# paolomandica/HALO

Measured on AMD Instinct MI355X. Metric: acquisition-scored images/sec (1024x2048, C=256, 19 cls), higher is better.
Workload: dtype f64

## Files before the change

### halo_amd/csrc/halo_score.hip

```cpp
#include "halo_common.hpp"
#include "halo_devmath.hpp"
#include "halo_select_plan.hpp"
#include "halo_softmax.hpp"
#include <stdlib.h>
#include <type_traits>

namespace halo {

constexpr int TPB = 256;
#ifndef HALO_FTPB
#define HALO_FTPB 128
#endif
#ifndef HALO_FEAT_WAVES
#define HALO_FEAT_WAVES 4
#endif
#ifndef HALO_FEAT_UNROLL
#define HALO_FEAT_UNROLL 8
#endif
#ifndef HALO_FEAT_STORE
#define HALO_FEAT_STORE 2
#endif
#ifndef HALO_FEAT_ENT_STORE
#define HALO_FEAT_ENT_STORE 1
#endif
// ... 765 lines not shown
    const int X0 = blockIdx.x * WB_TW, Y0 = blockIdx.y * WB_TH;
    const int nrows = H - Y0 < WB_TH ? H - Y0 : WB_TH, ncols = W - X0 < WB_TW ? W - X0 : WB_TW;
    const int Wt = WB_TW + 2 * r, Ht = nrows + 2 * r;
    const long long hw = (long long)H * W;
    const float *ep = ent + (size_t)b * hw;
    {
        const int tx = tid & 127;
        if (tx < Wt) {
            const int xs = tile_src(X0 + tx - r, W, X0 + ncols - 1, r, pad);
            for (int ty = tid >> 7; ty < Ht; ty += TPB / 128) {
                const int ys = tile_src(Y0 + ty - r, H, Y0 + nrows - 1, r, pad);
                tile[ty][tx] = (xs >= 0 && ys >= 0) ? ep[(size_t)ys * W + xs] : 0.0f;
            }
        }
    }
    __syncthreads();
    const int ry = tid & (WB_TH - 1), lx = (tid / WB_TH) * WB_P;
    const int y = Y0 + ry, xb = X0 + lx;
    const bool live = ry < nrows && lx < ncols;
    double mn = 0.0, mx = 0.0;
    if (live) {
        const int nfull = k >> 2, rem = k & 3;
        float acc[WB_P];
#pragma unroll
        for (int j = 0; j < WB_P; ++j) acc[j] = 0.0f;
        for (int dy = 0; dy < k; ++dy) {
            const float4 *row = reinterpret_cast<const float4 *>(&tile[ry + dy][lx]);
            float v[12];
            { const float4 q = row[0]; v[0] = q.x; v[1] = q.y; v[2] = q.z; v[3] = q.w; }
            { const float4 q = row[1]; v[4] = q.x; v[5] = q.y; v[6] = q.z; v[7] = q.w; }
            for (int c = 0; c < nfull; ++c) {
                { const float4 q = row[c + 2]; v[8] = q.x; v[9] = q.y; v[10] = q.z; v[11] = q.w; }
#pragma unroll
                for (int t = 0; t < 4; ++t)
#pragma unroll
                    for (int j = 0; j < WB_P; ++j) acc[j] = acc[j] + v[j + t];
#pragma unroll
                for (int i = 0; i < 8; ++i) v[i] = v[i + 4];
            }
#pragma unroll
            for (int j = 0; j < WB_P; ++j) acc[j] = acc[j] + v[j];
            if (rem == 3) {
                const float4 q = row[nfull + 2];
                v[8] = q.x; v[9] = q.y;
#pragma unroll
                for (int t = 1; t < 3; ++t)
#pragma unroll
                    for (int j = 0; j < WB_P; ++j) acc[j] = acc[j] + v[j + t];
            }
        }
        bool have = false;
#pragma unroll
        for (int j = 0; j < WB_P; ++j) {
            const int x = xb + j;
            if (x < W) {
                float cnt = 1.0f;
                if (pk > 0 && pad) {
                    cnt = (float)(pk * pk);
                } else if (pk > 0) {
                    const int pr = pk / 2;
                    const int y0 = y - pr < 0 ? 0 : y - pr, y1 = y + pr >= H ? H - 1 : y + pr;
                    const int x0 = x - pr < 0 ? 0 : x - pr, x1 = x + pr >= W ? W - 1 : x + pr;
                    cnt = (float)((y1 - y0 + 1) * (x1 - x0 + 1));
                }
                const float a = acc[j] / cnt;
                unc[(size_t)b * hw + (size_t)y * W + x] = a;
                if (!have) { mn = mx = (double)a; have = true; }
                else { mn = nan_min(mn, (double)a); mx = nan_max(mx, (double)a); }
            }
        }
    }
    if (!partials) return;
    __shared__ double seed[2];
    if (tid == 0) { seed[0] = mn; seed[1] = mx; }
    __syncthreads();
    if (!live) { mn = seed[0]; mx = seed[1]; }
    block_minmax<TPB>(mn, mx, partials + (((size_t)b * gridDim.y + blockIdx.y) * gridDim.x + blockIdx.x) * 2);
}

__device__ __forceinline__ float lane_prev(float v)
{
    return __int_as_float(__builtin_amdgcn_update_dpp(0, __float_as_int(v), 0x138 , 0xf, 0xf, false));
}
__device__ __forceinline__ float lane_next(float v)
{
    return __int_as_float(__builtin_amdgcn_update_dpp(0, __float_as_int(v), 0x130 , 0xf, 0xf, false));
}

__device__ __forceinline__ float box3_over_count(float a, int H, int W, int y, int xx, int pk)
{
    if (pk <= 0) return a;
    const int rr = pk / 2;
    const int y0 = y - rr < 0 ? 0 : y - rr, y1 = y + rr >= H ? H - 1 : y + rr;
    const int x0 = xx - rr < 0 ? 0 : xx - rr, x1 = xx + rr >= W ? W - 1 : xx + rr;
    return a / (float)((y1 - y0 + 1) * (x1 - x0 + 1));
}

__device__ __forceinline__ void box3_row4(const float *__restrict__ ep, int H, int W, int y, int x, bool live, int pk, float (&o)[4])
{
    const int lane = threadIdx.x & 63;
    float r[3][6];
#pragma unroll
    for (int dy = 0; dy < 3; ++dy) {
        const int yy = y + dy - 1;
        const bool in = live && yy >= 0 && yy < H;
        const float *row = ep + (size_t)(in ? yy : 0) * W;
        float4 q = make_float4(0.0f, 0.0f, 0.0f, 0.0f);
        if (in) q = *reinterpret_cast<const float4 *>(row + x);
        float left = lane_prev(q.w), right = lane_next(q.x);
        if (lane == 0) left = (in && x > 0) ? row[x - 1] : 0.0f;
        if (lane == 63) right = (in && x + 4 < W) ? row[x + 4] : 0.0f;
        r[dy][0] = (in && x > 0) ? left : 0.0f;
        r[dy][1] = q.x; r[dy][2] = q.y; r[dy][3] = q.z; r[dy][4] = q.w;
        r[dy][5] = (in && x + 4 < W) ? right : 0.0f;
    }
#pragma unroll
    for (int j = 0; j < 4; ++j) {
        float a = 0.0f;
#pragma unroll
        for (int dy = 0; dy < 3; ++dy)
#pragma unroll
            for (int dx = 0; dx < 3; ++dx) a = a + r[dy][j + dx];
        o[j] = box3_over_count(a, H, W, y, x + j, pk);
    }
}

__global__ void __launch_bounds__(TPB) k_box3_unc(const float *__restrict__ ent, int H, int W, int pk,
                                                  float *__restrict__ unc, double *__restrict__ partials)
{
    const int b = blockIdx.y;
    const long long hw = (long long)H * W;
    const long long i0 = ((long long)blockIdx.x * TPB + threadIdx.x) * 4;
    const bool live = i0 < hw;
    double mn = 0.0, mx = 0.0;
    const int y = live ? (int)(i0 / W) : 0, x = live ? (int)(i0 % W) : 0;
    float o[4];
    box3_row4(ent + (size_t)b * hw, H, W, y, x, live, pk, o);
    if (live) {
        if (unc) *reinterpret_cast<float4 *>(unc + (size_t)b * hw + i0) = make_float4(o[0], o[1], o[2], o[3]);
        mn = mx = (double)o[0];
#pragma unroll
        for (int j = 1; j < 4; ++j) { mn = nan_min(mn, (double)o[j]); mx = nan_max(mx, (double)o[j]); }
    }
    if (!partials) return;
    __shared__ double seed[2];
    if (threadIdx.x == 0) { seed[0] = mn; seed[1] = mx; }
    __syncthreads();
    if (!live) { mn = seed[0]; mx = seed[1]; }
    block_minmax<TPB>(mn, mx, partials + ((size_t)b * gridDim.x + blockIdx.x) * 2);
}

constexpr int BM_RPT = 4, BM_TW = 256, BM_TH = BM_RPT * (TPB / 64);

__device__ __forceinline__ float nan_minf(float a, float b) { return (a != a) ? a : ((b != b) ? b : (b < a ? b : a)); }
__device__ __forceinline__ float nan_maxf(float a, float b) { return (a != a) ? a : ((b != b) ? b : (b > a ? b : a)); }

__global__ void __launch_bounds__(TPB) k_box3_minmax(const float *__restrict__ ent, int H, int W, int pk, double *__restrict__ partials,
                                                     unsigned *__restrict__ hist_zero)
{
    const int b = blockIdx.z, lane = threadIdx.x & 63, wv = threadIdx.x >> 6;
    if (hist_zero) {
        const unsigned nb = gridDim.x * gridDim.y;
        for (unsigned l = blockIdx.y * gridDim.x + blockIdx.x; l < NB1 / TPB; l += nb) hist_zero[(size_t)b * NB1 + l * TPB + threadIdx.x] = 0u;
    }
    const int x = blockIdx.x * BM_TW + lane * 4, y0 = blockIdx.y * BM_TH + wv * BM_RPT;
    const float *ep = ent + (size_t)b * H * W;
    const bool xin = x < W;
    auto load_row = [&](int yy, float (&r)[6]) {
        const bool in = xin && yy >= 0 && yy < H;
        const float *row = ep + (size_t)(in ? yy : 0) * W;
        float4 q = make_float4(0.0f, 0.0f, 0.0f, 0.0f);
        if (in) q = *reinterpret_cast<const float4 *>(row + x);
        float left = lane_prev(q.w), right = lane_next(q.x);
        if (lane == 0) left = (in && x > 0) ? row[x - 1] : 0.0f;
        if (lane == 63) right = (in && x + 4 < W) ? row[x + 4] : 0.0f;
        r[0] = (in && x > 0) ? left : 0.0f;
        r[1] = q.x; r[2] = q.y; r[3] = q.z; r[4] = q.w;
        r[5] = (in && x + 4 < W) ? right : 0.0f;
    };
    float r0[6], r1[6], r2[6];
    load_row(y0 - 1, r0);
    load_row(y0, r1);
    float mn = 0.0f, mx = 0.0f;
    bool have = false;
#pragma unroll
    for (int k = 0; k < BM_RPT; ++k) {
        const int y = y0 + k;
        load_row(y + 1, r2);
        if (xin && y < H) {
#pragma unroll
            for (int j = 0; j < 4; ++j) {
                float a = 0.0f;
#pragma unroll
                for (int dx = 0; dx < 3; ++dx) a = a + r0[j + dx];
#pragma unroll
                for (int dx = 0; dx < 3; ++dx) a = a + r1[j + dx];
#pragma unroll
                for (int dx = 0; dx < 3; ++dx) a = a + r2[j + dx];
                const float o = box3_over_count(a, H, W, y, x + j, pk);
                if (!have) { mn = mx = o; have = true; }
                else { mn = nan_minf(mn, o); mx = nan_maxf(mx, o); }
            }
        }
#pragma unroll
        for (int q = 0; q < 6; ++q) { r0[q] = r1[q]; r1[q] = r2[q]; }
    }
    __shared__ float seedf[2];
    __shared__ float smn[TPB / 64], smx[TPB / 64];
    if (threadIdx.x == 0) { seedf[0] = mn; seedf[1] = mx; }
    __syncthreads();
    if (!have) { mn = seedf[0]; mx = seedf[1]; }
#pragma unroll
    for (int off = 32; off > 0; off >>= 1) {
        mn = nan_minf(mn, __shfl_xor(mn, off));
        mx = nan_maxf(mx, __shfl_xor(mx, off));
    }
    if (lane == 0) { smn[wv] = mn; smx[wv] = mx; }
    __syncthreads();
    if (threadIdx.x == 0) {
#pragma unroll
        for (int i = 1; i < TPB / 64; ++i) { mn = nan_minf(mn, smn[i]); mx = nan_maxf(mx, smx[i]); }
        double *out2 = partials + (((size_t)b * gridDim.y + blockIdx.y) * gridDim.x + blockIdx.x) * 2;
        out2[0] = (double)mn;
        out2[1] = (double)mx;
    }
}

__global__ void __launch_bounds__(TPB) k_minmax_f32(const float *__restrict__ x, long long hw,
                                                    double *__restrict__ partials)
{
    const int b = blockIdx.y;
    const long long i = (long long)blockIdx.x * TPB + threadIdx.x;
    const bool live = i < hw;
    double mn = 0.0, mx = 0.0;
    if (live) mn = mx = (double)x[(size_t)b * hw + i];
    __shared__ double seed[2];
    if (threadIdx.x == 0) { seed[0] = mn; seed[1] = mx; }
    __syncthreads();
    if (!live) { mn = seed[0]; mx = seed[1]; }
    block_minmax<TPB>(mn, mx, partials + ((size_t)b * gridDim.x + blockIdx.x) * 2);
}

__global__ void __launch_bounds__(TPB) k_fill_f32(float *__restrict__ x, long long n, float v)
{
    const long long i = (long long)blockIdx.x * TPB + threadIdx.x;
    if (i < n) x[i] = v;
}

template <typename TI>
__global__ void __launch_bounds__(TPB) k_combine(const TI *__restrict__ imp_raw, const float *__restrict__ unc_raw,
                                                 const double *__restrict__ stats, const unsigned char *__restrict__ active,
                                                 long long hw, int normalize, TI *__restrict__ score,
                                                 TI *__restrict__ imp_out, float *__restrict__ unc_out)
{
    const int b = blockIdx.y;
    const long long i = (long long)blockIdx.x * TPB + threadIdx.x;
    if (i >= hw) return;
    const size_t o = (size_t)b * hw + i;
    TI im = imp_raw[o];
    float un = unc_raw[o];
    if (normalize) {
        const float umn = (float)stats[b * 4 + 2], umx = (float)stats[b * 4 + 3];
        un = (un - umn) / (float)((double)umx - (double)umn);
        const TI imn = (TI)stats[b * 4 + 0], imx = (TI)stats[b * 4 + 1];
        if constexpr (sizeof(TI) == 8) im = (im - imn) / (imx - imn);
        else im = (im - imn) / (float)((double)imx - (double)imn);
    }
    TI s = im * (TI)un;
    if (active && active[o]) {
        if constexpr (sizeof(TI) == 8) s = __longlong_as_double(0xfff0000000000000ll);
        else s = __uint_as_float(0xff800000u);
    }
    score[o] = s;
    if (imp_out) imp_out[o] = im;
    if (unc_out) unc_out[o] = un;
}


constexpr int CB_ROWS = 16;

template <typename TI>
__global__ void __launch_bounds__(TPB) k_combine_box3(const TI *__restrict__ imp_raw, const float *__restrict__ ent,
                                                      const double *__restrict__ stats, const unsigned char *__restrict__ active,
                                                      int H, int W, int pk, int normalize, TI *__restrict__ score,
                                                      TI *__restrict__ imp_out, float *__restrict__ unc_out, SelHdr *__restrict__ rng,
                                                      unsigned *__restrict__ hist, int rows)
{
    __shared__ unsigned hl[NB1];
    const int b = blockIdx.z;
    const long long hw = (long long)H * W;
    const int x = (blockIdx.x * TPB + threadIdx.x) * 4;
    const bool live = x < W;
    float umn = 0.0f, uden = 1.0f;
    TI imn = (TI)0, iden = (TI)1;
    bool fin = false;
    if (normalize) {
        umn = (float)stats[b * 4 + 2];
        const float umx = (float)stats[b * 4 + 3];
        uden = (float)((double)umx - (double)umn);
        imn = (TI)stats[b * 4 + 0];
        const TI imx = (TI)stats[b * 4 + 1];
        if constexpr (sizeof(TI) == 8) iden = imx - imn;
        else iden = (float)((double)imx - (double)imn);
        fin = uden > 0.0f && uden < __builtin_inff() && iden > (TI)0 && iden < (TI)__builtin_inf();
        if (rng && blockIdx.x == 0 && blockIdx.y == 0 && threadIdx.x == 0) {
            SelHdr h;
            memset(&h, 0, sizeof(h));
            h.kmin_inv = ~order_key(0.0);
            h.kmax = order_key(1.0);
            h.nvalid = 1u;
            h.flags = fin ? (hist ? (unsigned)SEL_F_HIST : 0u) : (unsigned)SEL_F_BAD;
            rng[b] = h;
        }
    }
    const bool count = hist != nullptr && fin;
    if (count) {
        for (int j = threadIdx.x; j < NB1; j += TPB) hl[j] = 0u;
        __syncthreads();
    }
    ValRange vr;
    vr.lo = 0.0; vr.scale = (double)NB1; vr.ok = true;
    const int ybeg = blockIdx.y * rows, yend = ybeg + rows < H ? ybeg + rows : H;
    const float *ep = ent + (size_t)b * hw;
    const int lane = threadIdx.x & 63;
    struct RowRaw { float4 q; float el, er; bool in; };
    auto row_issue = [&](int yy) {
        RowRaw t;
        t.in = live && yy >= 0 && yy < H;
        const float *row = ep + (size_t)(t.in ? yy : 0) * W;
        t.q = make_float4(0.0f, 0.0f, 0.0f, 0.0f);
        t.el = 0.0f; t.er = 0.0f;
        if (t.in) t.q = *reinterpret_cast<const float4 *>(row + x);
        if (lane == 0 && t.in && x > 0) t.el = row[x - 1];
        if (lane == 63 && t.in && x + 4 < W) t.er = row[x + 4];
        return t;
    };
    auto row_finish = [&](const RowRaw &t, float (&r)[6]) {
        float left = lane_prev(t.q.w), right = lane_next(t.q.x);
        if (lane == 0) left = t.el;
        if (lane == 63) right = t.er;
        r[0] = (t.in && x > 0) ? left : 0.0f;
        r[1] = t.q.x; r[2] = t.q.y; r[3] = t.q.z; r[4] = t.q.w;
        r[5] = (t.in && x + 4 < W) ? right : 0.0f;
    };
    typedef double cb_d2 __attribute__((ext_vector_type(2)));
    typedef float cb_f4 __attribute__((ext_vector_type(4)));
    struct PixRaw { cb_d2 d0, d1; cb_f4 f; unsigned am; };
    auto pix_issue = [&](int yy) {
        PixRaw t;
        t.d0 = (cb_d2){0.0, 0.0}; t.d1 = t.d0; t.f = (cb_f4){0.f, 0.f, 0.f, 0.f}; t.am = 0u;
        if (!live || yy >= yend) return t;
        const size_t o = (size_t)b * hw + (size_t)yy * W + x;
        if constexpr (sizeof(TI) == 8) {
            t.d0 = *reinterpret_cast<const cb_d2 *>(imp_raw + o);
            t.d1 = *reinterpret_cast<const cb_d2 *>(imp_raw + o + 2);
        } else {
            t.f = *reinterpret_cast<const cb_f4 *>(imp_raw + o);
        }
        if (active) t.am = *reinterpret_cast<const unsigned *>(active + o);
        return t;
    };
    float r0[6], r1[6], r2[6];
    {
        const RowRaw a0 = row_issue(ybeg - 1), a1 = row_issue(ybeg);
        row_finish(a0, r0);
        row_finish(a1, r1);
    }
    RowRaw nrow = row_issue(ybeg + 1);
    PixRaw npix = pix_issue(ybeg);
    for (int y = ybeg; y < yend; ++y) {
        row_finish(nrow, r2);
        const PixRaw cpix = npix;
        nrow = row_issue(y + 2);
        npix = pix_issue(y + 1);
        float un[4];
#pragma unroll
        for (int j = 0; j < 4; ++j) {
            float a = 0.0f;
#pragma unroll
            for (int dx = 0; dx < 3; ++dx) a = a + r0[j + dx];
#pragma unroll
            for (int dx = 0; dx < 3; ++dx) a = a + r1[j + dx];
#pragma unroll
            for (int dx = 0; dx < 3; ++dx) a = a + r2[j + dx];
            un[j] = box3_over_count(a, H, W, y, x + j, pk);
        }
#pragma unroll
        for (int q = 0; q < 6; ++q) { r0[q] = r1[q]; r1[q] = r2[q]; }
        if (!live) continue;
        const size_t o = (size_t)b * hw + (size_t)y * W + x;
        TI im[4];
        if constexpr (sizeof(TI) == 8) { im[0] = cpix.d0.x; im[1] = cpix.d0.y; im[2] = cpix.d1.x; im[3] = cpix.d1.y; }
        else { im[0] = cpix.f.x; im[1] = cpix.f.y; im[2] = cpix.f.z; im[3] = cpix.f.w; }
        if (normalize) {
#pragma unroll
            for (int j = 0; j < 4; ++j) { un[j] = (un[j] - umn) / uden; im[j] = (im[j] - imn) / iden; }
        }
        const unsigned am = cpix.am;
        TI sc[4];
#pragma unroll
        for (int j = 0; j < 4; ++j) {
            sc[j] = im[j] * (TI)un[j];
            if ((am >> (8 * j)) & 0xffu) {
                if constexpr (sizeof(TI) == 8) sc[j] = __longlong_as_double(0xfff0000000000000ll);
                else sc[j] = __uint_as_float(0xff800000u);
            }
        }
        if (count) {
#pragma unroll
            for (int j = 0; j < 4; ++j) {
                const double v = (double)sc[j];
                const unsigned long long k = order_key(v);
                if (k < KEY_POS_INF && k != KEY_NEG_INF) {
                    double t;
                    atomicAdd(&hl[coarse_bin(v, vr, t)], 1u);
                }
            }
        }
        if constexpr (sizeof(TI) == 8) {
            *reinterpret_cast<double2 *>(score + o) = make_double2(sc[0], sc[1]);
            *reinterpret_cast<double2 *>(score + o + 2) = make_double2(sc[2], sc[3]);
            if (imp_out) {
                *reinterpret_cast<double2 *>(imp_out + o) = make_double2(im[0], im[1]);
                *reinterpret_cast<double2 *>(imp_out + o + 2) = make_double2(im[2], im[3]);
            }
        } else {
            *reinterpret_cast<float4 *>(score + o) = make_float4(sc[0], sc[1], sc[2], sc[3]);
            if (imp_out) *reinterpret_cast<float4 *>(imp_out + o) = make_float4(im[0], im[1], im[2], im[3]);
        }
        if (unc_out) *reinterpret_cast<float4 *>(unc_out + o) = make_float4(un[0], un[1], un[2], un[3]);
    }
    if (count) {
        __syncthreads();
        unsigned *g = hist + (size_t)b * NB1;
        for (int j = threadIdx.x; j < NB1; j += TPB)
            if (hl[j]) atomicAdd(&g[j], hl[j]);
    }
}



constexpr int LR_STAGE_IT = 3, LR_STAGE_G = 4;
constexpr int LR_TW = 64, LR_TH = 16, LR_PPT = 4;

template <typename T, int NPX = LR_PPT> struct LrW { T lx0, lx1, ly0[NPX], ly1[NPX]; };

struct LrTile { unsigned id; int b, X0, Y0; };
template <int TH> __device__ __forceinline__ LrTile lr_tile()
{
    const unsigned ntx = gridDim.x, nty = gridDim.y, ntiles = ntx * nty * gridDim.z;
    const unsigned lin = blockIdx.x + ntx * (blockIdx.y + nty * blockIdx.z);
    const unsigned xq = ntiles / 8, xr = ntiles % 8, xk = lin % 8;
    const unsigned id = (xk < xr ? xk * (xq + 1) : xr * (xq + 1) + (xk - xr) * xq) + lin / 8;
    return {id, (int)(id / (ntx * nty)), (int)(id % ntx) * LR_TW, (int)((id / ntx) % nty) * TH};
// ... 998 lines not shown
    p.pad = (a.flags >> 8) & 3;
    p.normalize = a.flags & HALO_FLAG_NORMALIZE;
    p.hw = (long long)a.H * a.W;
    p.nblk1 = (int)cdiv(p.hw, TPB);
    p.nblk_imp = p.nblk_unc = p.nblk1;

    Arena ar(a.workspace, a.workspace_bytes);
    p.ent = ar.take<float>(B * p.hw);
    p.unc_raw = ar.take<float>(B * p.hw);
    p.imp_raw = ar.take<double>(B * p.hw);
    p.pred = ar.take<short>(B * p.hw);
    p.part_imp = ar.take<double>(B * partial_slots(a.H, a.W) * 2);
    p.part_unc = ar.take<double>(B * partial_slots(a.H, a.W) * 2);
    p.stats = ar.take<double>(B * 4);
    p.lr_logit_full = (p.lr && !(a.O == 19 || a.O == 16)) ? ar.take<float>(B * a.O * p.hw) : nullptr;
    const bool gram_mode = a.route == HALO_SCORE_LR_GRAM && p.need_feat;
    if (gram_mode && a.feat_dtype != HALO_F64) return fail(HALO_E_UNSUPPORTED, "halo_score: float64 embeddings only on the Gram route");
    p.gram = gram_mode ? ar.take<double>(B * GRAM_MAPS * a.hf * a.wf) : nullptr;
    if (!ar.ok()) return fail(HALO_E_WORKSPACE, "halo_score: workspace too small");

    p.f64out = (a.pur_type == HALO_PUR_RADIUS || a.pur_type == HALO_PUR_EUC_NORM) && a.feat_dtype == HALO_F64;
    p.hist = is_ripu(a.pur_type) || a.pur_type == HALO_PUR_HYPER;
    p.mode = a.pur_type == HALO_PUR_EUC_NORM ? 1 : 0;
    p.ks = sqrt(fabs(-a.c) + 1e-15);
    p.rks = 1.0 / p.ks;

    const bool ent_only = (a.unc_type == HALO_UNC_ENTROPY || a.unc_type == HALO_UNC_PIXEL_ENTROPY) && !is_ripu(a.pur_type);
    const int fvec = !p.need_feat ? 0 : (a.feat_dtype == HALO_F64
        ? (((p.hw % 2 == 0) && (a.feat_bstride % 2 == 0) && aligned16(a.feat) && aligned16(p.imp_raw)) ? 2 : 1)
        : (((p.hw % 4 == 0) && (a.feat_bstride % 4 == 0) && aligned16(a.feat) && aligned16(p.imp_raw)) ? 4 : 1));
    p.fuse = !p.lr && p.need_feat && ent_only && (a.O == 19 || a.O == 16) && fvec > 1 && (a.logit_bstride % fvec == 0) &&
             (((uintptr_t)a.logit) % (4 * fvec) == 0);
    p.fl = FusedLogit{a.logit, (long long)a.logit_bstride, (int)a.O, a.unc_type, p.ent};
    return HALO_OK;
}

static void launch_logit_pass(const halo_score_args &a, const ScorePlan &p, hipStream_t st)
{
    if (p.fuse) return;
    const int B = (int)a.B, O = (int)a.O, H = (int)a.H, W = (int)a.W;
    const long long hw = p.hw, bstride = a.logit_bstride;
    const long long *gt = (const long long *)a.gt;
    short *pred = is_ripu(a.pur_type) ? p.pred : nullptr;
    const dim3 block(TPB), grid1((unsigned)p.nblk1, (unsigned)B);
    if (a.unc_type == HALO_UNC_ZEROS && !is_ripu(a.pur_type)) {
        hipLaunchKernelGGL(k_fill_f32, dim3((unsigned)cdiv(B * hw, TPB)), block, 0, st, p.ent, (long long)(B * hw), 0.0f);
    } else if (p.lr) {
        const int hl = (int)a.hl, wl = (int)a.wl;
        const float shl = H > 1 ? (float)(hl - 1) / (float)(H - 1) : 0.0f, swl = W > 1 ? (float)(wl - 1) / (float)(W - 1) : 0.0f;
        if (O == 19)
            hipLaunchKernelGGL((k_logit_maps_lr<19>), grid1, block, 0, st, a.logit, bstride, hl, wl, H, W, shl, swl, gt, a.unc_type, a.pur_type, p.ent, pred);
        else if (O == 16)
            hipLaunchKernelGGL((k_logit_maps_lr<16>), grid1, block, 0, st, a.logit, bstride, hl, wl, H, W, shl, swl, gt, a.unc_type, a.pur_type, p.ent, pred);
        else {
            hipLaunchKernelGGL(k_logit_interp_lr, grid1, block, 0, st, a.logit, bstride, O, hl, wl, H, W, shl, swl, p.lr_logit_full);
            hipLaunchKernelGGL(k_logit_maps_generic, grid1, block, 0, st, (const float *)p.lr_logit_full, (long long)(O * hw), gt, O, hw, a.unc_type, a.pur_type, 0, p.ent, pred);
        }
    } else {
        const bool vec4 = (hw % 4 == 0) && (bstride % 4 == 0) && aligned16(a.logit) && aligned16(p.ent);
        const dim3 grid4((unsigned)cdiv(hw, TPB * 4), (unsigned)B);
        if (O == 19 && vec4)
            hipLaunchKernelGGL((k_logit_maps<19, 4>), grid4, block, 0, st, a.logit, bstride, gt, hw, a.unc_type, a.pur_type, p.ent, pred);
        else if (O == 16 && vec4)
            hipLaunchKernelGGL((k_logit_maps<16, 4>), grid4, block, 0, st, a.logit, bstride, gt, hw, a.unc_type, a.pur_type, p.ent, pred);
        else
            hipLaunchKernelGGL(k_logit_maps_generic, grid1, block, 0, st, a.logit, bstride, gt, O, hw, a.unc_type, a.pur_type, 0, p.ent, pred);
    }
}

static void launch_gram(const halo_score_args &a, const ScorePlan &p, hipStream_t st)
{
    const double *feat = (const double *)a.feat;
    const long long bstride = a.feat_bstride;
    const int B = (int)a.B, C = (int)a.C, H = (int)a.H, W = (int)a.W, hf = (int)a.hf, wf = (int)a.wf;
    const dim3 block(TPB);
    const bool wide = wf >= 2 && wf % 2 == 0 && bstride % 2 == 0 && aligned16(feat) && aligned16(p.gram);
    if (wide) {
        const long long nwx = cdiv(wf, 128);
        int rows = 2;
        for (int cand = 8; cand > 2; cand >>= 1)
            if (B * nwx * cdiv(hf, cand) >= 1024) { rows = cand; break; }
        const long long nwaves = nwx * cdiv(hf, rows);
        const dim3 gg((unsigned)(cdiv(cdiv(nwaves, TPB / 64), 8) * 8), (unsigned)B);
#define HALO_GRAM2(U_, R_) hipLaunchKernelGGL((k_gram_lr2<U_, R_>), gg, block, 0, st, feat, bstride, C, hf, wf, p.gram)
        if (rows == 8) HALO_GRAM2(1, 8);
        else if (rows == 4) HALO_GRAM2(2, 4);
        else HALO_GRAM2(2, 2);
#undef HALO_GRAM2
    } else {
        const long long nwaves = cdiv(wf, GRAM_COLS) * cdiv(hf, 2);
        hipLaunchKernelGGL(k_gram_lr, dim3((unsigned)(cdiv(cdiv(nwaves, TPB / 64), 8) * 8), (unsigned)B), block, 0, st, feat, bstride, C, hf, wf, p.gram);
    }
    record(a.ev_feat_mid, st);
    const double shd = H > 1 ? (double)(hf - 1) / (double)(H - 1) : 0.0, swd = W > 1 ? (double)(wf - 1) / (double)(W - 1) : 0.0;
    const dim3 grid1((unsigned)p.nblk1, (unsigned)B);
    if (p.mode == 0) hipLaunchKernelGGL(k_radius_gram<0>, grid1, block, 0, st, p.gram, feat, bstride, C, hf, wf, H, W, shd, swd, p.ks, p.rks, p.imp_raw, p.part_imp);
    else hipLaunchKernelGGL(k_radius_gram<1>, grid1, block, 0, st, p.gram, feat, bstride, C, hf, wf, H, W, shd, swd, p.ks, p.rks, p.imp_raw, p.part_imp);
}

static int launch_feature_pass(const halo_score_args &a, ScorePlan &p, hipStream_t st)
{
    const int B = (int)a.B, C = (int)a.C;
    const long long hw = p.hw, bstride = a.feat_bstride;
    if (p.gram) {
        launch_gram(a, p, st);
        p.nblk_imp = p.nblk1;
    } else if (p.lr) {
        return a.feat_dtype == HALO_F64 ? launch_feat_lr<double>(a, p, p.imp_raw, st)
                                        : launch_feat_lr<float>(a, p, (float *)p.imp_raw, st);
    } else if (a.feat_dtype == HALO_F64) {
        const bool v2 = (hw % 2 == 0) && (bstride % 2 == 0) && aligned16(a.feat) && aligned16(p.imp_raw);
        p.nblk_imp = (int)cdiv(hw, v2 ? FTPB * 2 : FTPB);
        if (v2) launch_feat<double, 2>((const double *)a.feat, bstride, C, hw, B, p.mode, p.ks, p.rks, p.imp_raw, p.part_imp, p.nblk_imp, st, p.fuse ? &p.fl : nullptr);
        else launch_feat<double, 1>((const double *)a.feat, bstride, C, hw, B, p.mode, p.ks, p.rks, p.imp_raw, p.part_imp, p.nblk_imp, st, nullptr);
    } else {
        const bool v4 = (hw % 4 == 0) && (bstride % 4 == 0) && aligned16(a.feat) && aligned16(p.imp_raw);
        p.nblk_imp = (int)cdiv(hw, v4 ? FTPB * 4 : FTPB);
        if (v4) launch_feat<float, 4>((const float *)a.feat, bstride, C, hw, B, p.mode, p.ks, p.rks, (float *)p.imp_raw, p.part_imp, p.nblk_imp, st, p.fuse ? &p.fl : nullptr);
        else launch_feat<float, 1>((const float *)a.feat, bstride, C, hw, B, p.mode, p.ks, p.rks, (float *)p.imp_raw, p.part_imp, p.nblk_imp, st, nullptr);
    }
    return HALO_OK;
}

static int launch_tail(const halo_score_args &a, ScorePlan &p, hipStream_t st)
{
    const int64_t B = a.B, H = a.H, W = a.W;
    const long long hw = p.hw;
    const int normalize = p.normalize, box_pk = p.hist ? a.pksize : 0;
    const dim3 block(TPB), grid1((unsigned)p.nblk1, (unsigned)B);
    if (a.pur_type == HALO_PUR_HYPER) {
        hipLaunchKernelGGL(k_minmax_finalize, dim3((unsigned)B), block, 0, st, p.part_imp, p.nblk_imp, p.stats, 0);
        if (a.feat_dtype == HALO_F64) hipLaunchKernelGGL((k_quantize<double, short>), grid1, block, 0, st, (const double *)p.imp_raw, p.stats, hw, (int)a.K, p.pred);
        else hipLaunchKernelGGL((k_quantize<float, short>), grid1, block, 0, st, (const float *)p.imp_raw, p.stats, hw, (int)a.K, p.pred);
    }
    if (p.hist) {
        const float logK = (float)log((double)(a.pur_type == HALO_PUR_HYPER ? a.K : a.O));
        const int np = launch_region_impurity<short>((const short *)p.pred, B, H, W, a.pksize, a.pur_type == HALO_PUR_HYPER ? a.K : a.O, logK, (float *)p.imp_raw, (float *)nullptr, st,
                                                     normalize ? p.part_imp : nullptr, p.pad);
        p.nblk_imp = np ? np : p.nblk1;
        if (normalize && !np) hipLaunchKernelGGL(k_minmax_f32, grid1, block, 0, st, (const float *)p.imp_raw, hw, p.part_imp);
    } else if (a.pur_type == HALO_PUR_NONE) {
        hipLaunchKernelGGL(k_fill_f32, dim3((unsigned)cdiv(B * hw, TPB)), block, 0, st, (float *)p.imp_raw, (long long)(B * hw), 0.0f);
        if (normalize) hipLaunchKernelGGL(k_minmax_f32, grid1, block, 0, st, (const float *)p.imp_raw, hw, p.part_imp);
        p.nblk_imp = p.nblk1;
    }

    const int do_box = (a.unc_type == HALO_UNC_ENTROPY || a.unc_type == HALO_UNC_ORACLE_ACC) ? 1 : 0;
    const int box_route = do_box ? window_route(HALO_WINDOW_BOX, a.ksize, p.pad, 0, H, W) : 0;
    const bool box3 = box_route == 1 && aligned16(p.ent) && aligned16(p.unc_raw);
    const bool fuse_tail = box3 && B <= 65535 && H <= 65535 && aligned16(p.imp_raw) && aligned16(a.score) && (!a.impurity || aligned16(a.impurity)) &&
                           (!a.uncertainty || aligned16(a.uncertainty)) && (!a.active || ((uintptr_t)a.active & 3) == 0);
    SelHdr *rng_free = (a.score_range && normalize && fuse_tail) ? (SelHdr *)a.score_range : nullptr;
    unsigned *rng_hist = rng_free ? (unsigned *)((char *)a.score_range + range_hist_offset(B)) : nullptr;
    if (fuse_tail) {
        if (normalize) {
            const dim3 gridm((unsigned)cdiv(W, BM_TW), (unsigned)cdiv(H, BM_TH), (unsigned)B);
            p.nblk_unc = (int)(gridm.x * gridm.y);
            hipLaunchKernelGGL(k_box3_minmax, gridm, block, 0, st, (const float *)p.ent, (int)H, (int)W, box_pk, p.part_unc, rng_hist);
        }
    } else if (box3) {
        p.nblk_unc = (int)cdiv(hw, TPB * 4);
        hipLaunchKernelGGL(k_box3_unc, dim3((unsigned)p.nblk_unc, (unsigned)B), block, 0, st, (const float *)p.ent, (int)H, (int)W, box_pk, p.unc_raw,
                           normalize ? p.part_unc : nullptr);
    } else if (box_route == 2) {
        const dim3 gridw((unsigned)cdiv(W, WB_TW), (unsigned)cdiv(H, WB_TH), (unsigned)B);
        p.nblk_unc = (int)(gridw.x * gridw.y);
        hipLaunchKernelGGL(k_box_unc_tiled, gridw, block, 0, st, (const float *)p.ent, (int)H, (int)W, a.ksize, box_pk, p.unc_raw,
                           normalize ? p.part_unc : nullptr, p.pad);
    } else {
        hipLaunchKernelGGL(k_box_unc, grid1, block, 0, st, p.ent, (int)H, (int)W, a.ksize, do_box, box_pk, p.unc_raw, normalize ? p.part_unc : nullptr, p.pad);
    }

    if (normalize)
        hipLaunchKernelGGL(k_minmax_finalize2, dim3((unsigned)B, 2u), dim3(FIN_TPB), 0, st, (const double *)p.part_imp, p.nblk_imp,
                           (const double *)p.part_unc, p.nblk_unc, p.stats);
    if (fuse_tail) {
        int crows = CB_ROWS;
        while (crows > 1 && cdiv(W, TPB * 4) * cdiv(H, crows) * B < 1024) crows >>= 1;
        dim3 gridc((unsigned)cdiv(W, TPB * 4), (unsigned)cdiv(H, crows), (unsigned)B);
#define HALO_CB(T) hipLaunchKernelGGL((k_combine_box3<T>), gridc, block, 0, st, (const T *)p.imp_raw, (const float *)p.ent, p.stats, a.active, (int)H, (int)W, box_pk, normalize, (T *)a.score, (T *)a.impurity, a.uncertainty, rng_free, rng_hist, crows)
        if (p.f64out) HALO_CB(double);
        else HALO_CB(float);
#undef HALO_CB
    } else if (p.f64out) hipLaunchKernelGGL((k_combine<double>), grid1, block, 0, st, (const double *)p.imp_raw, p.unc_raw, p.stats, a.active, hw, normalize, (double *)a.score, (double *)a.impurity, a.uncertainty);
    else hipLaunchKernelGGL((k_combine<float>), grid1, block, 0, st, (const float *)p.imp_raw, p.unc_raw, p.stats, a.active, hw, normalize, (float *)a.score, (float *)a.impurity, a.uncertainty);
    if (a.score_range && !rng_free) {
        const int rc = score_range_exact(a.score, p.f64out ? HALO_F64 : HALO_F32, B, hw, a.score_range, st);
        if (rc != HALO_OK) return rc;
    }
    record(a.ev_tail_stop, st);
    return check_launch("halo_score");
}

static int score_impl(const halo_score_args &a, hipStream_t st)
{
    ScorePlan p;
    int rc = check_score_args(a);
    if (rc == HALO_OK) rc = make_score_plan(a, p);
    if (rc != HALO_OK) return rc;

    record(a.ev_logit_start, st);
    launch_logit_pass(a, p, st);
    record(a.ev_logit_stop, st);
    if (p.need_feat) {
        record(a.ev_feat_start, st);
        rc = launch_feature_pass(a, p, st);
        if (rc != HALO_OK) return rc;
        record(a.ev_feat_stop, st);
    }
    if (a.tail_stream && (hipStream_t)a.tail_stream != st) {
        if (!p.need_feat || !a.ev_feat_stop) return fail(HALO_E_ARG, "halo_score: a purity type that reads decoder_out and ev_feat_stop are required with a tail stream");
        if (hipStreamWaitEvent((hipStream_t)a.tail_stream, (hipEvent_t)a.ev_feat_stop, 0) != hipSuccess)
            return fail(HALO_E_LAUNCH, "halo_score: hipStreamWaitEvent: %s", hipGetErrorString(hipGetLastError()));
        st = (hipStream_t)a.tail_stream;
    }
    return launch_tail(a, p, st);
}

extern "C" int halo_score(const halo_score_args *a, void *stream)
{
    if (!a) return fail(HALO_E_ARG, "halo_score: null descriptor");
    return score_impl(*a, (hipStream_t)stream);
}

extern "C" int halo_region_uncertainty(const float *x, int64_t bstride, int is_prob, const int64_t *gt, int64_t B, int64_t O,
                                       int64_t H, int64_t W, int unc_type, int ksize, int do_box, float *out,
                                       void *workspace, size_t workspace_bytes, void *stream)
{
    hipStream_t st = (hipStream_t)stream;
    const int pad = (do_box >> 8) & 3;
    do_box &= 1;
    if (!x || !out || B <= 0 || O <= 0 || H <= 0 || W <= 0) return fail(HALO_E_ARG, "halo_region_uncertainty: null/empty argument");
    if (unc_type < 0 || unc_type > HALO_UNC_ZEROS) return fail(HALO_E_ARG, "halo_region_uncertainty: bad unc_type");
    if (unc_type == HALO_UNC_ORACLE_ACC && !gt) return fail(HALO_E_ARG, "halo_region_uncertainty: ground_truth required");
    if (ksize < 1 || !(ksize & 1)) return fail(HALO_E_ARG, "halo_region_uncertainty: window size must be odd");
    if (do_box) { const int rc = check_padding(pad, ksize, H, W, "halo_region_uncertainty"); if (rc != HALO_OK) return rc; }
    const long long hw = (long long)H * W;
    if (!workspace || workspace_bytes < (size_t)B * hw * 4 + 256) return fail(HALO_E_WORKSPACE, "halo_region_uncertainty: workspace too small");
    float *ent = (float *)(((uintptr_t)workspace + 255) & ~(uintptr_t)255);
    dim3 block(TPB), grid1((unsigned)cdiv(hw, TPB), (unsigned)B);
    float *dst = do_box ? ent : out;
    if (unc_type == HALO_UNC_ZEROS)
        hipLaunchKernelGGL(k_fill_f32, dim3((unsigned)cdiv(B * hw, TPB)), block, 0, st, dst, (long long)(B * hw), 0.0f);
    else
        hipLaunchKernelGGL(k_logit_maps_generic, grid1, block, 0, st, x, (long long)bstride, (const long long *)gt, (int)O, hw,
                           unc_type, HALO_PUR_NONE, is_prob, dst, (short *)nullptr);
    if (do_box && window_route(HALO_WINDOW_BOX, ksize, pad, 0, H, W) == 2)
        hipLaunchKernelGGL(k_box_unc_tiled, dim3((unsigned)cdiv(W, WB_TW), (unsigned)cdiv(H, WB_TH), (unsigned)B), block, 0, st, (const float *)ent,
                           (int)H, (int)W, ksize, 0, out, (double *)nullptr, pad);
    else if (do_box)
        hipLaunchKernelGGL(k_box_unc, grid1, block, 0, st, (const float *)ent, (int)H, (int)W, ksize, 1, 0, out, (double *)nullptr, pad);
    return check_launch("halo_region_uncertainty");
}

extern "C" int halo_region_impurity(const int64_t *pred, int64_t B, int64_t H, int64_t W, int ksize, int64_t K, float *impurity,
                                    float *count, int pad_mode, void *stream)
{
    if (!pred || !impurity || B <= 0 || H <= 0 || W <= 0 || K < 1) return fail(HALO_E_ARG, "halo_region_impurity: null/empty argument");
    if (ksize < 1 || !(ksize & 1)) return fail(HALO_E_ARG, "halo_region_impurity: window size must be odd");
    { const int rc = check_padding(pad_mode, ksize, H, W, "halo_region_impurity"); if (rc != HALO_OK) return rc; }
    launch_region_impurity<long long>((const long long *)pred, B, H, W, ksize, K, (float)log((double)K), impurity, count, (hipStream_t)stream,
                                      nullptr, pad_mode);
    return check_launch("halo_region_impurity");
}

extern "C" int halo_window_route(int what, int ksize, int pad_mode, int64_t bins, int64_t H, int64_t W)
{
    if (what != HALO_WINDOW_BOX && what != HALO_WINDOW_HIST) return fail(HALO_E_ARG, "halo_window_route: unknown window pass %d", what);
    if (ksize < 1 || !(ksize & 1)) return fail(HALO_E_ARG, "halo_window_route: window size must be odd");
    if (pad_mode < HALO_PAD_ZEROS || pad_mode > HALO_PAD_CIRCULAR) return fail(HALO_E_ARG, "halo_window_route: bad padding mode %d", pad_mode);
    if (H <= 0 || W <= 0) return fail(HALO_E_ARG, "halo_window_route: empty map");
    return window_route(what, ksize, pad_mode, bins, H, W);
}

extern "C" int halo_quantize_radius(const void *feat, int feat_dtype, int64_t feat_bstride, int64_t B, int64_t C, int64_t H,
                                    int64_t W, int64_t K, double c, int64_t *pred, void *workspace, size_t workspace_bytes,
                                    void *stream)
{
    hipStream_t st = (hipStream_t)stream;
    if (!feat || !pred || B <= 0 || C <= 0 || H <= 0 || W <= 0 || K < 1) return fail(HALO_E_ARG, "halo_quantize_radius: null/empty argument");
    if (feat_dtype != HALO_F32 && feat_dtype != HALO_F64) return fail(HALO_E_ARG, "halo_quantize_radius: bad dtype");
    if (!workspace || workspace_bytes < halo_score_workspace_bytes(B, H, W)) return fail(HALO_E_WORKSPACE, "halo_quantize_radius: workspace too small");
    const long long hw = (long long)H * W;
    const int nblk1 = (int)cdiv(hw, TPB), nblkf = (int)cdiv(hw, FTPB);
    Arena ar(workspace, workspace_bytes);
    double *imp_raw = ar.take<double>((size_t)B * hw);
    double *part = ar.take<double>((size_t)B * nblkf * 2);
    double *stats = ar.take<double>((size_t)B * 4);
    if (!ar.ok()) return fail(HALO_E_WORKSPACE, "halo_quantize_radius: workspace too small");
    const double ks = sqrt(fabs(-c) + 1e-15), rks = 1.0 / ks;
    dim3 block(TPB), grid1((unsigned)nblk1, (unsigned)B);
    if (feat_dtype == HALO_F64) {
        launch_feat<double, 1>((const double *)feat, feat_bstride, (int)C, hw, (int)B, 0, ks, rks, imp_raw, part, nblkf, st, nullptr);
        hipLaunchKernelGGL(k_minmax_finalize, dim3((unsigned)B), block, 0, st, (const double *)part, nblkf, stats, 0);
        hipLaunchKernelGGL((k_quantize<double, long long>), grid1, block, 0, st, (const double *)imp_raw, (const double *)stats, hw, (int)K, (long long *)pred);
    } else {
        launch_feat<float, 1>((const float *)feat, feat_bstride, (int)C, hw, (int)B, 0, ks, rks, (float *)imp_raw, part, nblkf, st, nullptr);
        hipLaunchKernelGGL(k_minmax_finalize, dim3((unsigned)B), block, 0, st, (const double *)part, nblkf, stats, 0);
        hipLaunchKernelGGL((k_quantize<float, long long>), grid1, block, 0, st, (const float *)imp_raw, (const double *)stats, hw, (int)K, (long long *)pred);
    }
    return check_launch("halo_quantize_radius");
}
```

Before: 1387.

## Fuse impurity min/max reduction into box3 kernel and drop finalize launch

The box3 min/max kernel now also reduces a slice of the impurity partials and writes combined per-block records. The combine kernel reduces those records itself, which removes the separate finalize kernel launch. The strip loader is also restructured: DPP lane shifts, software-prefetched rows, interior/edge template specialisation, a compile-time path for the pk case, and cheaper NaN tracking with fmin/fmax plus an any-NaN flag. In exchange, every combine block redundantly re-reduces all records, and NaN propagation semantics change subtly.

```diff
diff --git a/halo_amd/csrc/halo_score.hip b/halo_amd/csrc/halo_score.hip
--- a/halo_amd/csrc/halo_score.hip
+++ b/halo_amd/csrc/halo_score.hip
@@ -941,77 +941,167 @@
 
 constexpr int BM_RPT = 4, BM_TW = 256, BM_TH = BM_RPT * (TPB / 64);
 
-__device__ __forceinline__ float nan_minf(float a, float b) { return (a != a) ? a : ((b != b) ? b : (b < a ? b : a)); }
-__device__ __forceinline__ float nan_maxf(float a, float b) { return (a != a) ? a : ((b != b) ? b : (b > a ? b : a)); }
-
+__device__ __forceinline__ float lane_prev_or(float end, float v)
+{
+    return __int_as_float(__builtin_amdgcn_update_dpp(__float_as_int(end), __float_as_int(v), 0x138 , 0xf, 0xf, false));
+}
+__device__ __forceinline__ float lane_next_or(float end, float v)
+{
+    return __int_as_float(__builtin_amdgcn_update_dpp(__float_as_int(end), __float_as_int(v), 0x130 , 0xf, 0xf, false));
+}
+
+struct StripLane {
+    const float *ep;
+    int H, W, pk;
+    int x;
+    int xq, xe;
+    bool has_left, has_right;
+};
+
+constexpr int BM_AHEAD = 6;
+struct StripRaw { float4 q; float e; };
+
+template <bool INNER>
+__device__ __forceinline__ StripRaw strip_issue(const StripLane &s, int yy)
+{
+    StripRaw t;
+    t.q = make_float4(0.0f, 0.0f, 0.0f, 0.0f);
+    t.e = 0.0f;
+    if (INNER || (yy >= 0 && yy < s.H)) {
+        const float *row = s.ep + (size_t)yy * s.W;
+        t.q = *reinterpret_cast<const float4 *>(row + s.xq);
+        t.e = row[s.xe];
+    }
+    return t;
+}
+__device__ __forceinline__ void strip_finish(const StripLane &s, const StripRaw &t, float (&r)[6])
+{
+    const float left = lane_prev_or(t.e, t.q.w), right = lane_next_or(t.e, t.q.x);
+    r[0] = s.has_left ? left : 0.0f;
+    r[1] = t.q.x; r[2] = t.q.y; r[3] = t.q.z; r[4] = t.q.w;
+    r[5] = s.has_right ? right : 0.0f;
+}
+
+template <int R, bool INNER, bool PK>
+__device__ __forceinline__ void strip_rows(const StripLane &s, int y0, float &mn, float &mx, bool &nan)
+{
+    constexpr int D = R + 2 < BM_AHEAD ? R + 2 : BM_AHEAD;
+    StripRaw raw[D];
+#pragma unroll
+    for (int i = 0; i < D; ++i) raw[i] = strip_issue<INNER>(s, y0 - 1 + i);
+    float r0[6], r1[6], r2[6];
+    strip_finish(s, raw[0], r0);
+    if (D <= R + 1) raw[0] = strip_issue<INNER>(s, y0 - 1 + D);
+    strip_finish(s, raw[1 % D], r1);
+    if (1 + D <= R + 1) raw[1 % D] = strip_issue<INNER>(s, y0 + D);
+#pragma unroll
+    for (int k = 0; k < R; ++k) {
+        const int y = y0 + k;
+        if (!INNER && y >= s.H) break;
+        strip_finish(s, raw[(k + 2) % D], r2);
+        if (k + 2 + D <= R + 1) raw[(k + 2) % D] = strip_issue<INNER>(s, y + 1 + D);
+        float o[4];
+#pragma unroll
+        for (int j = 0; j < 4; ++j) {
+            float a = 0.0f;
+#pragma unroll
+            for (int dx = 0; dx < 3; ++dx) a = a + r0[j + dx];
+#pragma unroll
+            for (int dx = 0; dx < 3; ++dx) a = a + r1[j + dx];
+#pragma unroll
+            for (int dx = 0; dx < 3; ++dx) a = a + r2[j + dx];
+            o[j] = PK ? box3_over_count(a, s.H, s.W, y, s.x + j, s.pk) : a;
+        }
+        mn = __builtin_fminf(__builtin_fminf(mn, o[0]), __builtin_fminf(o[1], __builtin_fminf(o[2], o[3])));
+        mx = __builtin_fmaxf(__builtin_fmaxf(mx, o[0]), __builtin_fmaxf(o[1], __builtin_fmaxf(o[2], o[3])));
+        nan = nan | __builtin_isunordered(o[0], o[1]) | __builtin_isunordered(o[2], o[3]);
+#pragma unroll
+        for (int q = 0; q < 6; ++q) { r0[q] = r1[q]; r1[q] = r2[q]; }
+    }
+}
+
+template <bool PK>
 __global__ void __launch_bounds__(TPB) k_box3_minmax(const float *__restrict__ ent, int H, int W, int pk, double *__restrict__ partials,
-                                                     unsigned *__restrict__ hist_zero)
-{
-    const int b = blockIdx.z, lane = threadIdx.x & 63, wv = threadIdx.x >> 6;
+                                                     unsigned *__restrict__ hist_zero, const double *__restrict__ part_imp, int nimp)
+{
+    const int b = blockIdx.z, lane = threadIdx.x & 63, wv = __builtin_amdgcn_readfirstlane(threadIdx.x >> 6);
     if (hist_zero) {
         const unsigned nb = gridDim.x * gridDim.y;
         for (unsigned l = blockIdx.y * gridDim.x + blockIdx.x; l < NB1 / TPB; l += nb) hist_zero[(size_t)b * NB1 + l * TPB + threadIdx.x] = 0u;
     }
-    const int x = blockIdx.x * BM_TW + lane * 4, y0 = blockIdx.y * BM_TH + wv * BM_RPT;
-    const float *ep = ent + (size_t)b * H * W;
-    const bool xin = x < W;
-    auto load_row = [&](int yy, float (&r)[6]) {
-        const bool in = xin && yy >= 0 && yy < H;
-        const float *row = ep + (size_t)(in ? yy : 0) * W;
-        float4 q = make_float4(0.0f, 0.0f, 0.0f, 0.0f);
-        if (in) q = *reinterpret_cast<const float4 *>(row + x);
-        float left = lane_prev(q.w), right = lane_next(q.x);
-        if (lane == 0) left = (in && x > 0) ? row[x - 1] : 0.0f;
-        if (lane == 63) right = (in && x + 4 < W) ? row[x + 4] : 0.0f;
-        r[0] = (in && x > 0) ? left : 0.0f;
-        r[1] = q.x; r[2] = q.y; r[3] = q.z; r[4] = q.w;
-        r[5] = (in && x + 4 < W) ? right : 0.0f;
-    };
-    float r0[6], r1[6], r2[6];
-    load_row(y0 - 1, r0);
-    load_row(y0, r1);
-    float mn = 0.0f, mx = 0.0f;
-    bool have = false;
-#pragma unroll
-    for (int k = 0; k < BM_RPT; ++k) {
-        const int y = y0 + k;
-        load_row(y + 1, r2);
-        if (xin && y < H) {
-#pragma unroll
-            for (int j = 0; j < 4; ++j) {
-                float a = 0.0f;
-#pragma unroll
-                for (int dx = 0; dx < 3; ++dx) a = a + r0[j + dx];
-#pragma unroll
-                for (int dx = 0; dx < 3; ++dx) a = a + r1[j + dx];
-#pragma unroll
-                for (int dx = 0; dx < 3; ++dx) a = a + r2[j + dx];
-                const float o = box3_over_count(a, H, W, y, x + j, pk);
-                if (!have) { mn = mx = o; have = true; }
-                else { mn = nan_minf(mn, o); mx = nan_maxf(mx, o); }
-            }
-        }
-#pragma unroll
-        for (int q = 0; q < 6; ++q) { r0[q] = r1[q]; r1[q] = r2[q]; }
-    }
-    __shared__ float seedf[2];
+    const unsigned S = gridDim.x * gridDim.y, wg = blockIdx.y * gridDim.x + blockIdx.x;
+    double imn = 0.0, imx = 0.0;
+    int inan = 0;
+    if (part_imp) {
+        const double2 *pi = reinterpret_cast<const double2 *>(part_imp) + (size_t)b * nimp;
+        const unsigned each = (unsigned)nimp / S, more = (unsigned)nimp % S;
+        const unsigned i0 = wg * each + (wg < more ? wg : more), i1 = i0 + each + (wg < more ? 1u : 0u);
+        const double2 first = pi[i0 < i1 ? i0 : 0];
+        imn = first.x; imx = first.y;
+        inan = (imn != imn ? 1 : 0) | (imx != imx ? 2 : 0);
+        for (unsigned i = i0 + threadIdx.x; i < i1; i += TPB) {
+            const double2 q = pi[i];
+            inan |= (q.x != q.x ? 1 : 0) | (q.y != q.y ? 2 : 0);
+            imn = __builtin_fmin(imn, q.x); imx = __builtin_fmax(imx, q.y);
+        }
+    }
+    StripLane s;
+    s.ep = ent + (size_t)b * H * W;
+    s.H = H; s.W = W; s.pk = pk;
+    s.x = blockIdx.x * BM_TW + lane * 4;
+    const bool xin = s.x < W;
+    s.xq = xin ? s.x : W - 4;
+    s.has_left = xin && s.x > 0;
+    s.has_right = xin && s.x + 4 < W;
+    s.xe = lane == 0 ? (s.has_left ? s.x - 1 : 0) : (lane == 63 && s.has_right ? s.x + 4 : s.xq);
+    constexpr int R = BM_RPT;
+    const int y0 = blockIdx.y * BM_TH + wv * R;
+    float mn = __builtin_inff(), mx = -__builtin_inff();
+    bool nan = false;
+    if (y0 >= 1 && y0 + R < H) strip_rows<R, true, PK>(s, y0, mn, mx, nan);
+    else if (y0 < H) strip_rows<R, false, PK>(s, y0, mn, mx, nan);
+    if (!xin) { mn = __builtin_inff(); mx = -__builtin_inff(); nan = false; }
+#pragma unroll
+    for (int off = 32; off > 0; off >>= 1) {
+        mn = __builtin_fminf(mn, __shfl_xor(mn, off));
+        mx = __builtin_fmaxf(mx, __shfl_xor(mx, off));
+    }
+    const bool wnan = __any(nan) != 0;
+    int winan = 0;
+    if (part_imp) {
+#pragma unroll
+        for (int off = 32; off > 0; off >>= 1) {
+            imn = __builtin_fmin(imn, __shfl_xor(imn, off));
+            imx = __builtin_fmax(imx, __shfl_xor(imx, off));
+        }
+        winan = (__any(inan & 1) ? 1 : 0) | (__any(inan & 2) ? 2 : 0);
+    }
     __shared__ float smn[TPB / 64], smx[TPB / 64];
-    if (threadIdx.x == 0) { seedf[0] = mn; seedf[1] = mx; }
-    __syncthreads();
-    if (!have) { mn = seedf[0]; mx = seedf[1]; }
-#pragma unroll
-    for (int off = 32; off > 0; off >>= 1) {
-        mn = nan_minf(mn, __shfl_xor(mn, off));
-        mx = nan_maxf(mx, __shfl_xor(mx, off));
-    }
-    if (lane == 0) { smn[wv] = mn; smx[wv] = mx; }
+    __shared__ int snan[TPB / 64], sinan[TPB / 64];
+    __shared__ double simn[TPB / 64], simx[TPB / 64];
+    if (lane == 0) { smn[wv] = mn; smx[wv] = mx; snan[wv] = wnan; simn[wv] = imn; simx[wv] = imx; sinan[wv] = winan; }
     __syncthreads();
     if (threadIdx.x == 0) {
-#pragma unroll
-        for (int i = 1; i < TPB / 64; ++i) { mn = nan_minf(mn, smn[i]); mx = nan_maxf(mx, smx[i]); }
-        double *out2 = partials + (((size_t)b * gridDim.y + blockIdx.y) * gridDim.x + blockIdx.x) * 2;
-        out2[0] = (double)mn;
-        out2[1] = (double)mx;
+        bool bnan = wnan;
+#pragma unroll
+        for (int i = 1; i < TPB / 64; ++i) {
+            mn = __builtin_fminf(mn, smn[i]); mx = __builtin_fmaxf(mx, smx[i]); bnan = bnan | (snan[i] != 0);
+            imn = __builtin_fmin(imn, simn[i]); imx = __builtin_fmax(imx, simx[i]); winan |= sinan[i];
+        }
+        const double qnan = (double)__builtin_nanf("");
+        if (winan & 1) imn = qnan;
+        if (winan & 2) imx = qnan;
+        const double umn = bnan ? qnan : (double)mn;
+        const double umx = bnan ? qnan : (double)mx;
+        if (part_imp) {
+            double2 *rec = reinterpret_cast<double2 *>(partials) + ((size_t)b * S + wg) * 2;
+            rec[0] = make_double2(imn, imx);
+            rec[1] = make_double2(umn, umx);
+        } else {
+            double *out2 = partials + ((size_t)b * S + wg) * 2;
+            out2[0] = umn;
+            out2[1] = umx;
+        }
     }
 }
 
@@ -1070,10 +1160,10 @@
 
 template <typename TI>
 __global__ void __launch_bounds__(TPB) k_combine_box3(const TI *__restrict__ imp_raw, const float *__restrict__ ent,
-                                                      const double *__restrict__ stats, const unsigned char *__restrict__ active,
+                                                      double *__restrict__ stats, const unsigned char *__restrict__ active,
                                                       int H, int W, int pk, int normalize, TI *__restrict__ score,
                                                       TI *__restrict__ imp_out, float *__restrict__ unc_out, SelHdr *__restrict__ rng,
-                                                      unsigned *__restrict__ hist, int rows)
+                                                      unsigned *__restrict__ hist, int rows, const double *__restrict__ recs, int nrec)
 {
     __shared__ unsigned hl[NB1];
     const int b = blockIdx.z;
@@ -1084,11 +1174,40 @@
     TI imn = (TI)0, iden = (TI)1;
     bool fin = false;
     if (normalize) {
-        umn = (float)stats[b * 4 + 2];
-        const float umx = (float)stats[b * 4 + 3];
+        double st4[4];
+        if (recs) {
+            const double2 *rp = reinterpret_cast<const double2 *>(recs) + (size_t)b * nrec * 2;
+            const double2 a0 = rp[0], b0 = rp[1];
+            st4[0] = a0.x; st4[1] = a0.y; st4[2] = b0.x; st4[3] = b0.y;
+            int bad = 0;
+            for (int i = threadIdx.x & 63; i < nrec; i += 64) {
+                const double2 a = rp[2 * i], c = rp[2 * i + 1];
+                bad |= (a.x != a.x ? 1 : 0) | (a.y != a.y ? 2 : 0) | (c.x != c.x ? 4 : 0) | (c.y != c.y ? 8 : 0);
+                st4[0] = __builtin_fmin(st4[0], a.x); st4[1] = __builtin_fmax(st4[1], a.y);
+                st4[2] = __builtin_fmin(st4[2], c.x); st4[3] = __builtin_fmax(st4[3], c.y);
+            }
+#pragma unroll
+            for (int off = 32; off > 0; off >>= 1) {
+                st4[0] = __builtin_fmin(st4[0], __shfl_xor(st4[0], off)); st4[1] = __builtin_fmax(st4[1], __shfl_xor(st4[1], off));
+                st4[2] = __builtin_fmin(st4[2], __shfl_xor(st4[2], off)); st4[3] = __builtin_fmax(st4[3], __shfl_xor(st4[3], off));
+            }
+            const double qnan = (double)__builtin_nanf("");
+#pragma unroll
+            for (int k = 0; k < 4; ++k)
+                if (__any(bad & (1 << k))) st4[k] = qnan;
+            if (blockIdx.x == 0 && blockIdx.y == 0 && threadIdx.x == 0) {
+#pragma unroll
+                for (int k = 0; k < 4; ++k) stats[b * 4 + k] = st4[k];
+            }
+        } else {
+#pragma unroll
+            for (int k = 0; k < 4; ++k) st4[k] = stats[b * 4 + k];
+        }
+        umn = (float)st4[2];
+        const float umx = (float)st4[3];
         uden = (float)((double)umx - (double)umn);
-        imn = (TI)stats[b * 4 + 0];
-        const TI imx = (TI)stats[b * 4 + 1];
+        imn = (TI)st4[0];
+        const TI imx = (TI)st4[1];
         if constexpr (sizeof(TI) == 8) iden = imx - imn;
         else iden = (float)((double)imx - (double)imn);
         fin = uden > 0.0f && uden < __builtin_inff() && iden > (TI)0 && iden < (TI)__builtin_inf();
@@ -2393,11 +2512,15 @@
                            (!a.uncertainty || aligned16(a.uncertainty)) && (!a.active || ((uintptr_t)a.active & 3) == 0);
     SelHdr *rng_free = (a.score_range && normalize && fuse_tail) ? (SelHdr *)a.score_range : nullptr;
     unsigned *rng_hist = rng_free ? (unsigned *)((char *)a.score_range + range_hist_offset(B)) : nullptr;
+    bool records = false;
     if (fuse_tail) {
         if (normalize) {
             const dim3 gridm((unsigned)cdiv(W, BM_TW), (unsigned)cdiv(H, BM_TH), (unsigned)B);
             p.nblk_unc = (int)(gridm.x * gridm.y);
-            hipLaunchKernelGGL(k_box3_minmax, gridm, block, 0, st, (const float *)p.ent, (int)H, (int)W, box_pk, p.part_unc, rng_hist);
+            records = 2 * (int64_t)p.nblk_unc <= (int64_t)partial_slots(H, W);
+            const double *imp_pairs = records ? (const double *)p.part_imp : nullptr;
+            if (box_pk > 0) hipLaunchKernelGGL((k_box3_minmax<true>), gridm, block, 0, st, (const float *)p.ent, (int)H, (int)W, box_pk, p.part_unc, rng_hist, imp_pairs, p.nblk_imp);
+            else hipLaunchKernelGGL((k_box3_minmax<false>), gridm, block, 0, st, (const float *)p.ent, (int)H, (int)W, box_pk, p.part_unc, rng_hist, imp_pairs, p.nblk_imp);
         }
     } else if (box3) {
         p.nblk_unc = (int)cdiv(hw, TPB * 4);
@@ -2412,14 +2535,14 @@
         hipLaunchKernelGGL(k_box_unc, grid1, block, 0, st, p.ent, (int)H, (int)W, a.ksize, do_box, box_pk, p.unc_raw, normalize ? p.part_unc : nullptr, p.pad);
     }
 
-    if (normalize)
+    if (normalize && !records)
         hipLaunchKernelGGL(k_minmax_finalize2, dim3((unsigned)B, 2u), dim3(FIN_TPB), 0, st, (const double *)p.part_imp, p.nblk_imp,
                            (const double *)p.part_unc, p.nblk_unc, p.stats);
     if (fuse_tail) {
         int crows = CB_ROWS;
         while (crows > 1 && cdiv(W, TPB * 4) * cdiv(H, crows) * B < 1024) crows >>= 1;
         dim3 gridc((unsigned)cdiv(W, TPB * 4), (unsigned)cdiv(H, crows), (unsigned)B);
-#define HALO_CB(T) hipLaunchKernelGGL((k_combine_box3<T>), gridc, block, 0, st, (const T *)p.imp_raw, (const float *)p.ent, p.stats, a.active, (int)H, (int)W, box_pk, normalize, (T *)a.score, (T *)a.impurity, a.uncertainty, rng_free, rng_hist, crows)
+#define HALO_CB(T) hipLaunchKernelGGL((k_combine_box3<T>), gridc, block, 0, st, (const T *)p.imp_raw, (const float *)p.ent, p.stats, a.active, (int)H, (int)W, box_pk, normalize, (T *)a.score, (T *)a.impurity, a.uncertainty, rng_free, rng_hist, crows, records ? (const double *)p.part_unc : nullptr, p.nblk_unc)
         if (p.f64out) HALO_CB(double);
         else HALO_CB(float);
 #undef HALO_CB
```

Result: no change. 1390, median of 6 (+0.2%).
